# montekki/thaler-study

Hardware: AMD Instinct MI355X
Metric: field mul-adds/sec in sumcheck prover, n=28 vars (higher is better)
Workload: dtype u64

## Files before the change

thaler-study_amd/csrc/engine/abi_context.inc:

```


extern "C" int sc_field_from_modulus(uint64_t p, sc_field* out) {
  if (!out) return SC_ERR_ARG;
  sc::FieldParams fp;
  if (!sc::field_params_from_modulus(p, &fp)) return SC_ERR_ARG;
  out->p = fp.p;
  out->p_inv_neg = fp.p_inv_neg;
  out->r_mod_p = fp.r_mod_p;
  out->r2_mod_p = fp.r2_mod_p;
  return SC_OK;
}

static sc::FieldParams to_params(const sc_field* f) {
  sc::FieldParams fp;
  fp.p = f->p;
  fp.p_inv_neg = f->p_inv_neg;
  fp.r_mod_p = f->r_mod_p;
  fp.r2_mod_p = f->r2_mod_p;
  return fp;
}

extern "C" uint64_t sc_field_to_mont(const sc_field* f, uint64_t canonical) {
  HostField hf(to_params(f));
  return hf.mul(canonical % f->p, f->r2_mod_p);
// ... 73 lines not shown
  memset(ctx->h_tail, 0, kTailSlots * kTailSlotWords * sizeof(u64));
  SC_CREATE_HIP(hipHostGetDevicePointer((void**)&ctx->d_tail, ctx->h_tail, 0));
  for (int i = kTailSlots - 1; i >= 0; --i) ctx->tail_free.push_back(i);
  SC_CREATE_HIP(hipDeviceSynchronize());
  for (int i = 0; i < sc_ctx::kTimerRing; ++i) {
    SC_CREATE_HIP(hipEventCreate(&ctx->kt_ev[i][0]));
    SC_CREATE_HIP(hipEventCreate(&ctx->kt_ev[i][1]));
  }
#undef SC_CREATE_HIP
  *out = ctx;
  return SC_OK;
}

extern "C" int sc_ctx_destroy(sc_ctx* ctx) {
  if (!ctx) return SC_OK;
  if (is_multi(ctx)) return multi_destroy(ctx);
  (void)hipSetDevice(ctx->device);
  if (ctx->stream) (void)sync_stream(ctx);
  if (ctx->comm && g_rccl.CommDestroy) g_rccl.CommDestroy(ctx->comm);
  for (int q = 0; q < sc::kMaxPeers; ++q)
    if (ctx->peer_ipc_opened[q] && ctx->peer_base[q]) (void)hipIpcCloseMemHandle(ctx->peer_base[q]);
  if (ctx->peer_region) (void)hipFree(ctx->peer_region);
  for (auto& kv : ctx->pool_free) (void)hipFree(kv.second);
  for (auto& kv : ctx->pool_live) (void)hipFree(kv.first);
  if (ctx->d_partials) (void)hipFree(ctx->d_partials);
  if (ctx->d_wg_partials) (void)hipFree(ctx->d_wg_partials);
  if (ctx->d_wg_groups) (void)hipFree(ctx->d_wg_groups);
  if (ctx->d_wg_tickets) (void)hipFree(ctx->d_wg_tickets);
  if (ctx->d_gram_rows) (void)hipFree(ctx->d_gram_rows);
  if (ctx->d_sums) (void)hipFree(ctx->d_sums);
  if (ctx->h_sums) (void)hipHostFree(ctx->h_sums);
  if (ctx->h_mailbox) (void)hipHostFree(ctx->h_mailbox);
  if (ctx->h_tail) (void)hipHostFree(ctx->h_tail);
  if (ctx->h_points) (void)hipHostFree(ctx->h_points);
  if (ctx->d_points) (void)hipFree(ctx->d_points);
  for (u64* tw : ctx->d_rs_twiddles)
    if (tw) (void)hipFree(tw);
  for (u64* tw : ctx->d_rs_twist)
    if (tw) (void)hipFree(tw);
  if (ctx->d_xc_inv) (void)hipFree(ctx->d_xc_inv);
  if (ctx->h_batch_desc) (void)hipHostFree(ctx->h_batch_desc);
  if (ctx->h_batch) (void)hipHostFree(ctx->h_batch);
  if (ctx->d_ticket) (void)hipFree(ctx->d_ticket);
  for (int i = 0; i < sc_ctx::kTimerRing; ++i)
    for (int k = 0; k < 2; ++k)
      if (ctx->kt_ev[i][k]) (void)hipEventDestroy(ctx->kt_ev[i][k]);
  if (ctx->stream) (void)hipStreamDestroy(ctx->stream);
  delete ctx;
  return SC_OK;
}

extern "C" const char* sc_last_error(const sc_ctx* ctx) {
  return ctx ? ctx->err.c_str() : g_create_error.c_str();
}

static int prewarm(sc_ctx* ctx, size_t num_vars);

enum : unsigned { kOptBool = 1, kOptOff = 2, kOptPeer = 4 };
struct OptionSpec {
  const char* name;
  int sc_ctx::*member;
  int64_t lo, hi;
  unsigned flags;
};
const OptionSpec kOptions[] = {
    {"vars_per_pass", &sc_ctx::vars_per_pass, 1, 2, 0},
    {"first_pass_vars", &sc_ctx::first_pass_vars, 0, 4, 0},
    {"grid_pass", &sc_ctx::grid_pass, 0, 1, kOptBool},
    {"grid_log", &sc_ctx::grid_log, 0, 26, 0},
    {"grid_max_vars", &sc_ctx::grid_max_vars, 1, sc::kGridMaxVars, 0},
    {"grid_sharded", &sc_ctx::grid_sharded, 0, 1, kOptBool},
    {"grid_blocks", &sc_ctx::grid_blocks, 0, kWgMaxBlocks, 0},
    {"fold_dma", &sc_ctx::fold_dma, 0, 1, kOptBool},
    {"pipe32", &sc_ctx::pipe32, 0, 1, kOptBool},
    {"pipe32_log", &sc_ctx::pipe32_log, 11, 40, 0},
    {"gram_log", &sc_ctx::gram_log, 14, 40, kOptOff},
    {"wfold_log", &sc_ctx::wfold_log, 12, 40, kOptOff},
    {"wfold_min_log", &sc_ctx::wfold_min_log, 12, 40, 0},
    {"wfold5_min_log", &sc_ctx::wfold5_min_log, 12, 40, 0},
    {"wfold_always", &sc_ctx::wfold_always, 0, 1, kOptBool},
    {"wfold_slot_period", &sc_ctx::wfold_slot_period, -1, 1 << 24, 0},
    {"wfold_slot_width", &sc_ctx::wfold_slot_width, 0, 1 << 24, 0},
    {"wfold_slot_stagger", &sc_ctx::wfold_slot_stagger, 0, 1, kOptBool},
    {"matmul_path", &sc_ctx::matmul_path, 0, 2, 0},
    {"host_tail_log", &sc_ctx::host_tail_log, 0, kTailLogMax, 0},
    {"gp_host_log", &sc_ctx::gp_host_log, 0, sc::kGpHostLogMax, 0},
    {"gp_tree_lv", &sc_ctx::gp_tree_lv, 1, 3, 0},
    {"fr_host_log", &sc_ctx::fr_host_log, 0, sc::kFrHostLogMax, 0},
    {"fr_tree_lv", &sc_ctx::fr_tree_lv, 1, sc::kFrTreeLvMax, 0},
    {"tail_log", &sc_ctx::tail_log, 0, 40, 0},
    {"max_blocks", &sc_ctx::max_blocks, 1, INT64_MAX, 0},
    {"time_kernels", &sc_ctx::time_kernels, 0, 1, kOptBool},
    {"use_mailbox", &sc_ctx::use_mailbox, 0, 1, kOptBool},
    {"nt_load_log", &sc_ctx::nt_load_log, INT64_MIN, INT64_MAX, 0},
    {"nt_store_log", &sc_ctx::nt_store_log, INT64_MIN, INT64_MAX, 0},
    {"pool_contiguous", &sc_ctx::pool_contiguous, 0, 1, kOptBool},
    {"dbg_fold_grab", &sc_ctx::dbg_fold_grab, 0, 16, 0},
    {"rccl_timeout_ms", &sc_ctx::rccl_timeout_ms, 1, 3600000, 0},
    {"arena_log", &sc_ctx::arena_log, 4, 26, kOptPeer},
    {"peer_spin_ms", &sc_ctx::peer_spin_ms, 1, 600000, kOptPeer},
    {"peer_connect_ms", &sc_ctx::peer_connect_ms, 1, 3600000, kOptPeer},
    {"dbg_delay_ms", &sc_ctx::dbg_delay_ms, 0, 10000, kOptPeer},
    {"dbg_skip_tag", &sc_ctx::dbg_skip_tag, 0, 1, kOptBool | kOptPeer},
};
static const OptionSpec* find_option(const char* key) {
  for (const OptionSpec& o : kOptions)
    if (strcmp(o.name, key) == 0) return &o;
  return nullptr;
}

extern "C" int sc_ctx_set_option(sc_ctx* ctx, const char* key, int64_t value) {
  if (!ctx || !key) return SC_ERR_ARG;
  const std::string k(key);
  if (k == "prewarm") return value < 0 ? fail(ctx, SC_ERR_ARG, "prewarm: num_vars must be >= 0") : prewarm(ctx, (size_t)value);
  if (is_multi(ctx)) SC_TRY(multi_set_option(ctx, key, value));
  if (k == "stat_reset") {
    ctx->stat_wait_ns = ctx->stat_launch_ns = 0;
    ctx->pool_peak_words = ctx->pool_live_words;
    return SC_OK;
  }
  const OptionSpec* o = find_option(key);
  if (!o) return fail(ctx, SC_ERR_ARG, "unknown option '%s'", key);
  if (o->member == &sc_ctx::max_blocks && (value < 1 || value > (int64_t)ctx->partial_rows))
    return fail(ctx, SC_ERR_ARG, "max_blocks must be 1..%zu", ctx->partial_rows);
  if (!(o->flags & kOptBool) && (value < o->lo || value > o->hi) && !((o->flags & kOptOff) && value == 0))
    return fail(ctx, SC_ERR_ARG, "%s must be %s%lld..%lld", key, (o->flags & kOptOff) ? "0 (never) or " : "", (long long)o->lo, (long long)o->hi);
  if (o->member == &sc_ctx::arena_log && ctx->peer_region) return fail(ctx, SC_ERR_STATE, "arena_log must be set before sc_ctx_comm_peer_export");
  ctx->*o->member = (o->flags & kOptBool) ? (value ? 1 : 0) : (int)value;
  return SC_OK;
}

static int64_t pool_stat(const sc_ctx* ctx, size_t (*of)(const sc_ctx*)) {
  if (!is_multi(ctx)) return (int64_t)of(ctx);
  int64_t sum = 0;
  for (const sc_ctx* sub : ctx->subs) sum += (int64_t)of(sub);
  return sum;
}

extern "C" int sc_ctx_get_option(const sc_ctx* ctx, const char* key, int64_t* value) {
  if (!ctx || !key || !value) return SC_ERR_ARG;
  const std::string k(key);
  if (k == "stat_wait_ns") *value = (int64_t)(is_multi(ctx) ? ctx->subs[0]->stat_wait_ns : ctx->stat_wait_ns);
  else if (k == "stat_launch_ns") *value = (int64_t)(is_multi(ctx) ? ctx->subs[0]->stat_launch_ns : ctx->stat_launch_ns);
  else if (k == "stat_pool_live_blocks") *value = pool_stat(ctx, [](const sc_ctx* c) { return c->pool_live.size(); });
  else if (k == "stat_pool_live_words") *value = pool_stat(ctx, [](const sc_ctx* c) { return c->pool_live_words; });
  else if (k == "stat_pool_peak_words") *value = pool_stat(ctx, [](const sc_ctx* c) { return c->pool_peak_words; });
  else if (k == "transport") *value = (int64_t)ctx->transport;
  else if (k == "n_devices") *value = is_multi(ctx) ? (int64_t)ctx->subs.size() : 1;
  else if (k == "comm_nranks") {
    int n = ctx->world;
    if (ctx->transport == Transport::kRccl) {
      n = 0;
      if (!g_rccl.CommCount || !ctx->comm || g_rccl.CommCount(ctx->comm, &n) != ncclSuccess)
        return fail(ctx, SC_ERR_RCCL, "ncclCommCount failed");
    }
    *value = n;
  } else if (const OptionSpec* o = find_option(key)) {
    *value = ctx->*o->member;
  } else {
    return fail(ctx, SC_ERR_ARG, "unknown option '%s'", key);
  }
  return SC_OK;
}

extern "C" int sc_ctx_synchronize(sc_ctx* ctx) {
  if (!ctx) return SC_ERR_ARG;
  if (is_multi(ctx)) return multi_synchronize(ctx);
  SC_TRY(set_device(ctx));
  SC_HIP(ctx, sync_stream(ctx));
  return SC_OK;
}

extern "C" void* sc_ctx_stream(const sc_ctx* ctx) { return !ctx ? nullptr : (void*)(is_multi(ctx) ? ctx->subs[0]->stream : ctx->stream); }

extern "C" int sc_ctx_kernel_time(sc_ctx* ctx, double out[2], int reset) {
  if (!ctx || !out) return SC_ERR_ARG;
  if (is_multi(ctx)) {
    for (size_t d = 1; d < ctx->subs.size(); ++d) {
      double drop[2];
      (void)sc_ctx_kernel_time(ctx->subs[d], drop, reset);
    }
    return sc_ctx_kernel_time(ctx->subs[0], out, reset);
  }
  SC_TRY(set_device(ctx));
  drain_kernel_timers(ctx);
  out[0] = (double)ctx->kt_n;
  out[1] = ctx->kt_ms;
  if (reset) {
    ctx->kt_n = 0;
    ctx->kt_ms = 0.0;
  }
  return SC_OK;
}

extern "C" int sc_ctx_launch_log(sc_ctx* ctx, sc_launch_record* out, size_t cap, size_t* n_out, int reset) {
  if (!ctx || !n_out || (cap && !out)) return SC_ERR_ARG;
  if (is_multi(ctx)) {
    for (size_t d = 1; d < ctx->subs.size(); ++d) {
      size_t drop = 0;
      (void)sc_ctx_launch_log(ctx->subs[d], nullptr, 0, &drop, reset);
    }
    return sc_ctx_launch_log(ctx->subs[0], out, cap, n_out, reset);
  }
  SC_TRY(set_device(ctx));
  drain_kernel_timers(ctx);
  const size_t n = std::min(cap, ctx->launch_log.size());
  for (size_t i = 0; i < n; ++i) out[i] = ctx->launch_log[i];
  *n_out = ctx->launch_log.size();
  if (reset) ctx->launch_log.clear();
// ... 3 lines not shown
```

thaler-study_amd/csrc/engine/launch.inc:

```

namespace {


#define SC_DISPATCH_FIELD(ctx, F, f, ...)      \
  do {                                         \
    if ((ctx)->gold) {                         \
      typedef sc::GoldilocksMont F;            \
      F f((ctx)->fp);                          \
      __VA_ARGS__;                             \
    } else {                                   \
      typedef sc::MontGeneric F;               \
      F f((ctx)->fp);                          \
      __VA_ARGS__;                             \
    }                                          \
  } while (0)

template <int V>
using IntC = std::integral_constant<int, V>;
template <int... Vs, class Fn>
void with_const(int v, Fn&& fn) {
  (void)((v == Vs && (fn(IntC<Vs>{}), true)) || ...);
}
template <class Fn>
void with_bool(bool b, Fn&& fn) {
// ... 205 lines not shown
    SC_HIP(ctx, hipGetLastError());
  }
  ctx->mailbox_seq += 1;
  return SC_OK;
}

bool in_tail(const sc_ctx* ctx, const u64* p) { return p && ctx->d_tail && p >= ctx->d_tail && p < ctx->d_tail + kTailSlots * kTailSlotWords; }

int launch_pass(sc_ctx* ctx, int kf, int ks, const u64* A, const u64* B, u64* A2, u64* B2, const u64* r,
                int log_in, bool across_ranks, bool* from_mailbox) {
  if (kf < 0 || kf > 4 || ks < 1 || ks > 3 || (ks == 3 && kf != 0) || (kf == 4 && (ks != 2 || log_in < 12)) || log_in < kf + ks)
    return fail(ctx, SC_ERR_ARG, "launch_pass: kf=%d ks=%d log_in=%d", kf, ks, log_in);
  const sc::FoldW fw = make_weights<sc::FoldW>(ctx, r, kf);
  size_t n_units = (size_t)1 << (log_in - kf - ks);
  const bool pipe32 = kf == 3 && ks == 2 && ctx->pipe32 && n_units % sc::kWave == 0 && log_in >= ctx->pipe32_log;
  const size_t bs = (size_t)sc::pass_block_threads(kf, ks, pipe32 ? 4 : 0);
  int grid = (int)std::min<size_t>(std::max<size_t>((n_units + bs - 1) / bs, 1), (size_t)ctx->max_blocks);
  grid = std::min(grid, pipe32 ? pipe32_resident_blocks(ctx) : pass_resident_blocks(ctx, kf, ks));
  if (kf > 0 && in_tail(ctx, A2) && (grid != 1 || ((size_t)1 << (log_in - kf)) > (size_t)sc::kWave))
    return fail(ctx, SC_ERR_STATE, "launch_pass: a pass_kernel launch of %d blocks would hand 2^%d-entry tables to the host with plain stores", grid,
                log_in - kf);
  const sc::PassOut out = next_pass_out(ctx, across_ranks, challenge_digest(r, kf, ks, log_in), from_mailbox);
  SC_TRY(timer_begin(ctx, SC_KIND_PASS, kf, ks, log_in, (u64)16 << log_in, kf > 0 ? (u64)16 << (log_in - kf) : 0));
  SC_DISPATCH_FIELD(ctx, F, f, launch_pass_t<F>(ctx, f, kf, ks, A, B, A2, B2, fw, n_units, grid, log_in, out, pipe32));
  SC_TRY(commit_pass_out(ctx, out, grid));
  SC_TRY(timer_end(ctx));
  return SC_OK;
}

int wait_mailbox(sc_ctx* ctx, u64 seq);

int check_exchange(sc_ctx* ctx, const char* what) {
  const u64 err = __atomic_load_n(ctx->h_mailbox + sc::kMailboxErr, __ATOMIC_ACQUIRE);
  if (err == 0) return SC_OK;
  if (err & (u64)sc::kXchgTimeout) {
    poison(ctx);
    return fail(ctx, SC_ERR_RCCL, "peer exchange: a rank's %s did not arrive within %d ms (rank %d waited for rank %d at tag %u; that rank's "
                "slot held tag ..%04x)", what, ctx->peer_spin_ms, ctx->rank, (int)((err >> 8) & 0xFF), ctx->xchg_tag, (unsigned)((err >> 16) & 0x3FFF));
  }
  return fail(ctx, SC_ERR_STATE, "the ranks of this sharded prover were given different challenges");
}

int launch_grid_pass(sc_ctx* ctx, int kf, int ks, const u64* A, const u64* B, u64* A2, u64* B2, const u64* r, int log_in, bool across_ranks) {
  if (kf < 0 || kf > sc::kGridMaxVars || ks < 1 || ks > sc::kGridMaxVars || log_in < kf + ks)
    return fail(ctx, SC_ERR_ARG, "launch_grid_pass: kf=%d ks=%d log_in=%d", kf, ks, log_in);
  if (!ctx->use_mailbox) return fail(ctx, SC_ERR_STATE, "launch_grid_pass needs the host mailbox");
  const sc::GridW gw = make_weights<sc::GridW>(ctx, r, kf);
  const size_t n_out = (size_t)1 << (log_in - kf);
  const int resident = std::min(resident_grid(ctx, ctx->gold ? kernel_ptr(&sc::wgrid_pass_kernel<sc::GoldilocksMont, 5, false>)
                                                             : kernel_ptr(&sc::wgrid_pass_kernel<sc::MontGeneric, 5, false>),
                                              sc::kBlock, 2 * ctx->num_cus),
                                kWgMaxBlocks);
  constexpr size_t kWaves = sc::kBlock / sc::kWave;
  const size_t n_iter = (n_out + sc::kWgEntries - 1) / sc::kWgEntries;
  const size_t cap = ctx->grid_blocks > 0 ? (size_t)std::min(ctx->grid_blocks, resident) : (size_t)resident;
  const int grid = (int)std::max<size_t>(1, std::min<size_t>((n_iter + kWaves - 1) / kWaves, cap));
  const sc::WgOut wo = next_wide_out(ctx, across_ranks, challenge_digest(r, kf, ks, log_in), true, in_tail(ctx, A2));
  SC_TRY(timer_begin(ctx, SC_KIND_GRID_PASS, kf, ks, log_in, (u64)16 << log_in, kf > 0 ? (u64)16 << (log_in - kf) : 0));
  const bool pf = (kf == 0 || kf == 2) && n_iter > (size_t)grid * kWaves;
  SC_DISPATCH_FIELD(ctx, F, f, with_bool(pf, [&](auto PF) {
    with_const<1, 2, 3, 4, 5>(ks, [&](auto KS) {
      hipLaunchKernelGGL((sc::wgrid_pass_kernel<F, KS, PF>), dim3(grid), dim3(sc::kBlock), 0, ctx->stream, f, A, B, A2, B2, gw, kf, n_out, wo);
    });
  }));
  return commit_wide_out(ctx, wo, pow3(ks));
}
bool wfold_has(int kf, int ks) { return (kf == 4 && ks == 5) || (kf == 5 && ks >= 3 && ks <= 5); }
int wfold_resident_blocks(sc_ctx* ctx) {
  const void* fn = ctx->gold ? kernel_ptr(&sc::wfold_pass_kernel<sc::GoldilocksMont, 4, 5, true>)
                             : kernel_ptr(&sc::wfold_pass_kernel<sc::MontGeneric, 4, 5, true>);
  return std::min(resident_grid(ctx, fn, sc::kWfThreads, ctx->num_cus), kWgMaxBlocks);
}
int launch_wfold_pass(sc_ctx* ctx, int kf, int ks, const u64* A, const u64* B, u64* A2, u64* B2, const u64* r, int log_in, bool across_ranks) {
  if (log_in < 12 || !A2 || !B2 || !wfold_has(kf, ks)) return fail(ctx, SC_ERR_ARG, "launch_wfold_pass: kf=%d ks=%d log_in=%d", kf, ks, log_in);
  if (!ctx->use_mailbox) return fail(ctx, SC_ERR_STATE, "launch_wfold_pass needs the host mailbox");
  const sc::FoldW fw = make_weights<sc::FoldW>(ctx, r, 4);
  const u64 r_top = kf == 5 ? r[4] : 0;
  const size_t n_tiles = (size_t)1 << (log_in - 12);
  const int grid = (int)std::max<size_t>(1, std::min<size_t>(std::min<size_t>(n_tiles, (size_t)wfold_resident_blocks(ctx)), (size_t)ctx->max_blocks));
  const sc::WgOut wo = next_wide_out(ctx, across_ranks, challenge_digest(r, kf, ks, log_in) ^ 0x77666f6cu, true, false);
  SC_TRY(timer_begin(ctx, SC_KIND_WFOLD_PASS, kf, ks, log_in, (u64)16 << log_in, (u64)16 << (log_in - kf)));
  sc::WfSlots sl;
  if (ctx->wfold_slot_period < 0) {
    sl.period = (kf == 4 && log_in >= 25) ? 2400u : 0u;
    sl.width = 600u;
  } else {
    sl.period = (unsigned)ctx->wfold_slot_period;
    sl.width = (unsigned)ctx->wfold_slot_width;
    sl.stagger = (unsigned)ctx->wfold_slot_stagger;
  }
  SC_DISPATCH_FIELD(ctx, F, f, with_bool(log_in >= ctx->nt_load_log, [&](auto NT) {
    with_bool(sl.period != 0, [&](auto SLOTS) {
      auto go = [&](auto KF, auto KS) {
        hipLaunchKernelGGL((sc::wfold_pass_kernel<F, KF, KS, NT, SLOTS>), dim3(grid), dim3(sc::kWfThreads), 0, ctx->stream, f, A, B, A2, B2, fw, r_top,
                           n_tiles, wo, sl);
      };
      if (kf == 4) go(IntC<4>{}, IntC<5>{});
      else with_const<3, 4, 5>(ks, [&](auto KS) { go(IntC<5>{}, KS); });
    });
  }));
  return commit_wide_out(ctx, wo, pow3(ks));
}

constexpr int kGramK = 4;
constexpr int kGramMaxBlocks = 1024;
int gram_workspace(sc_ctx* ctx) {
  if (ctx->d_gram_rows) return SC_OK;
  const size_t bytes = (size_t)kGramMaxBlocks * sc::kGramRowWords * sizeof(u64) + 64;
  u64* p = nullptr;
  SC_HIP(ctx, hipMalloc(&p, bytes));
  hipError_t e = hipMemsetAsync(p, 0, bytes, ctx->stream);
  const int lds = sc::kGramStages * sc::kGramStageBytes;
  const void* fns[4] = {reinterpret_cast<const void*>(&sc::gram_pass_kernel<sc::GoldilocksMont, kGramK, true>),
                        reinterpret_cast<const void*>(&sc::gram_pass_kernel<sc::GoldilocksMont, kGramK, false>),
                        reinterpret_cast<const void*>(&sc::gram_pass_kernel<sc::MontGeneric, kGramK, true>),
                        reinterpret_cast<const void*>(&sc::gram_pass_kernel<sc::MontGeneric, kGramK, false>)};
  for (int i = 0; i < 4 && e == hipSuccess; ++i) e = hipFuncSetAttribute(fns[i], hipFuncAttributeMaxDynamicSharedMemorySize, lds);
  if (e != hipSuccess) {
    (void)hipFree(p);
    SC_HIP(ctx, e);
  }
  ctx->d_gram_rows = p;
  return SC_OK;
}
int launch_gram_pass(sc_ctx* ctx, const u64* A, const u64* B, int log_in, bool across_ranks) {
  typedef sc::GramGeo<kGramK> G;
  if (!ctx->use_mailbox) return fail(ctx, SC_ERR_STATE, "launch_gram_pass needs the host mailbox");
  const size_t len = (size_t)1 << log_in;
  if (len < (size_t)G::kEntriesPerStep * sc::kGramStages) return fail(ctx, SC_ERR_ARG, "launch_gram_pass: 2^%d entries are too few", log_in);
  const size_t n_steps = len / G::kEntriesPerStep;
  size_t blocks = 1;
  while (blocks * 2 <= (size_t)std::min(std::min(ctx->num_cus, ctx->max_blocks), kGramMaxBlocks)) blocks *= 2;
  size_t n_partials = std::min(blocks, n_steps / sc::kGramStages);
  while (n_steps / n_partials > (size_t)G::kMaxSteps) n_partials *= 2;
  const size_t spp = n_steps / n_partials;
  const int grid = (int)std::min(blocks, n_partials);
  SC_TRY(gram_workspace(ctx));
  const sc::WgOut wo = next_wide_out(ctx, across_ranks, challenge_digest(nullptr, 0, kGramK, log_in) ^ 0x6772616du, false, false);
  unsigned* ticket = reinterpret_cast<unsigned*>(ctx->d_gram_rows + (size_t)kGramMaxBlocks * sc::kGramRowWords);
  SC_TRY(timer_begin(ctx, SC_KIND_GRAM_PASS, 0, kGramK, log_in, (u64)16 << log_in, (u64)grid * sc::kGramRowWords * sizeof(u64)));
  const unsigned char* a8 = reinterpret_cast<const unsigned char*>(A);
  const unsigned char* b8 = reinterpret_cast<const unsigned char*>(B);
  const int lds = sc::kGramStages * sc::kGramStageBytes;
  SC_DISPATCH_FIELD(ctx, F, f, with_bool(log_in >= ctx->nt_load_log, [&](auto NT) {
    hipLaunchKernelGGL((sc::gram_pass_kernel<F, kGramK, NT>), dim3(grid), dim3(sc::kGramThreads), lds, ctx->stream, f, a8, b8,
                       (unsigned)n_partials, (unsigned)spp, ctx->d_gram_rows, ticket, wo);
  }));
  return commit_wide_out(ctx, wo, pow3(kGramK));
}

int collect_grid(sc_ctx* ctx, int ks, bool across_ranks, u64* out) {
  SC_TRY(wait_mailbox(ctx, ctx->mailbox_seq));
  const int cells = pow3(ks);
  const u64* wide = ctx->h_mailbox + sc::kMailboxWide;
  if (!across_ranks) {
    for (int c = 0; c < cells; ++c) out[c] = wide[c];
    return SC_OK;
  }
  HostField hf(ctx->fp);
  if (ctx->transport == Transport::kHost) {
    std::vector<u64> limbs(2 * (size_t)cells);
    for (int c = 0; c < cells; ++c) {
      limbs[2 * c] = wide[c] & 0xFFFFFFFFull;
      limbs[2 * c + 1] = wide[c] >> 32;
    }
    if (ctx->host_allreduce(ctx->host_user, limbs.data(), limbs.size()) != 0)
      return fail(ctx, SC_ERR_RCCL, "host all-reduce callback failed");
    for (int c = 0; c < cells; ++c) out[c] = hf.recombine(limbs[2 * c], limbs[2 * c + 1]);
    return SC_OK;
  }
  if (ctx->transport == Transport::kPeer) SC_TRY(check_exchange(ctx, "sums"));
  for (int c = 0; c < cells; ++c) out[c] = hf.recombine(wide[2 * c], wide[2 * c + 1]);
// ... 20 lines not shown
```

thaler-study_amd/csrc/kernels/grid_pass.hpp:

```cpp
#pragma once

namespace sc {

constexpr int kGridChunk = 256;
constexpr int kGridMaxVars = 5;
constexpr int kGridMaxCells = 243;
constexpr int kMailboxWide = 64;
constexpr int kMailboxWords = kMailboxWide + 512;
constexpr int kWgEntries = 32;
constexpr int kWgGroupBlocks = 32;
struct GridW {
  u64 w[1 << kGridMaxVars];
};
struct WgOut {
  u64* partials;
  u64* group_rows;
  unsigned* tickets;
  u64* mailbox;
  u64 seq;
  u64* limbs_dev;
  PeerX px;
  int host_out = 0;
};
template <class F, int KF>
// ... 279 lines not shown
    return;
  }
  if (tid < CELLS) __hip_atomic_store(out.mailbox + kMailboxWide + tid, total, __ATOMIC_RELAXED, __HIP_MEMORY_SCOPE_SYSTEM);
  asm volatile("s_waitcnt vmcnt(0)" ::: "memory");
  __syncthreads();
  if (tid == 0) __hip_atomic_store(out.mailbox + kMailboxSeq, out.seq, __ATOMIC_RELEASE, __HIP_MEMORY_SCOPE_SYSTEM);
}

template <class F, int KS>
__device__ __forceinline__ void wgrid_finish(const F& f, u64 total, const WgOut& out) {
  constexpr int kPow3[6] = {1, 3, 9, 27, 81, 243};
  constexpr int cells = kPow3[KS];
  __shared__ int lds_flag;
  const int tid = threadIdx.x;
  if (gridDim.x > 1) {
    const int n_blocks = gridDim.x, group = blockIdx.x / kWgGroupBlocks, n_groups = (n_blocks + kWgGroupBlocks - 1) / kWgGroupBlocks;
    const int group_size = min(kWgGroupBlocks, n_blocks - group * kWgGroupBlocks);
    if (tid < cells)
      __hip_atomic_store(out.partials + (size_t)blockIdx.x * kGridChunk + tid, total, __ATOMIC_RELAXED, __HIP_MEMORY_SCOPE_AGENT);
    asm volatile("s_waitcnt vmcnt(0)" ::: "memory");
    __syncthreads();
    if (tid == 0) {
      const unsigned t = __hip_atomic_fetch_add(out.tickets + 1 + group, 1u, __ATOMIC_RELAXED, __HIP_MEMORY_SCOPE_AGENT);
      const int last = (t == (unsigned)group_size - 1) ? 1 : 0;
      if (last) {
        __builtin_amdgcn_fence(__ATOMIC_ACQUIRE, "agent");
        asm volatile("s_waitcnt vmcnt(0)" ::: "memory");
      }
      lds_flag = last;
    }
    __syncthreads();
    if (!lds_flag) return;
    total = 0;
    if (tid < cells) {
      u64 x[kWgGroupBlocks];
#pragma unroll
      for (int q = 0; q < kWgGroupBlocks; ++q)
        x[q] = (q < group_size) ? __hip_atomic_load(out.partials + (size_t)(group * kWgGroupBlocks + q) * kGridChunk + tid, __ATOMIC_RELAXED,
                                                    __HIP_MEMORY_SCOPE_AGENT)
                                : 0;
#pragma unroll
      for (int q = 0; q < kWgGroupBlocks; ++q) total = f.add(total, x[q]);
    }
    if (n_groups > 1) {
      __syncthreads();
      if (tid < cells)
        __hip_atomic_store(out.group_rows + (size_t)group * kGridChunk + tid, total, __ATOMIC_RELAXED, __HIP_MEMORY_SCOPE_AGENT);
      asm volatile("s_waitcnt vmcnt(0)" ::: "memory");
      __syncthreads();
      if (tid == 0) {
        const unsigned t = __hip_atomic_fetch_add(out.tickets, 1u, __ATOMIC_RELAXED, __HIP_MEMORY_SCOPE_AGENT);
        const int last = (t == (unsigned)n_groups - 1) ? 1 : 0;
        if (last) {
          __builtin_amdgcn_fence(__ATOMIC_ACQUIRE, "agent");
          asm volatile("s_waitcnt vmcnt(0)" ::: "memory");
        }
        lds_flag = last;
      }
      __syncthreads();
      if (!lds_flag) return;
      total = 0;
      if (tid < cells) {
        u64 x[kWgGroupBlocks];
#pragma unroll
        for (int q = 0; q < kWgGroupBlocks; ++q)
          x[q] = (q < n_groups) ? __hip_atomic_load(out.group_rows + (size_t)q * kGridChunk + tid, __ATOMIC_RELAXED, __HIP_MEMORY_SCOPE_AGENT) : 0;
#pragma unroll
        for (int q = 0; q < kWgGroupBlocks; ++q) total = f.add(total, x[q]);
      }
    }
    if (tid <= n_groups) __hip_atomic_store(out.tickets + tid, 0u, __ATOMIC_RELAXED, __HIP_MEMORY_SCOPE_AGENT);
  }
  publish_cells<cells>(out, total);
}

template <class F, int KS, bool PF>
__global__ void __launch_bounds__(kBlock)
wgrid_pass_kernel(F f, const u64* __restrict__ A, const u64* __restrict__ B, u64* __restrict__ A2, u64* __restrict__ B2,
                  GridW gw, int kf, size_t n_out, WgOut out) {
  const u64 total = wgrid_body<F, KS, PF>(f, A, B, A2, B2, gw, kf, n_out, out.host_out != 0);
  wgrid_finish<F, KS>(f, total, out);
}

#define SC_WFOLD_SLOTS 1
struct WfSlots {
  unsigned period = 0;
  unsigned width = 0;
  unsigned stagger = 0;
};
constexpr int kWfThreads = 512;
template <class F, int KF, int KS, bool NT, bool SLOTS = false>
__global__ void __launch_bounds__(kWfThreads)
wfold_pass_kernel(F f, const u64* __restrict__ A, const u64* __restrict__ B, u64* __restrict__ A2, u64* __restrict__ B2, FoldW fw,
                  u64 r_top, size_t n_tiles, WgOut out, WfSlots sl) {
  static_assert(KF == 4 || KF == 5, "four or five pending challenges");
  static_assert(KS >= 1 && KS <= 5, "one to five rounds");
  constexpr int OUT = 4, NPS = 8, NP = 32;
  constexpr int OUTS = kWave >> (KF - 4);
  constexpr int TILE_OUT = OUT * OUTS;
  constexpr int NPO = TILE_OUT / (2 * kWave);
  constexpr int kWaves = kWfThreads / kWave;
  constexpr int kPow3[6] = {1, 3, 9, 27, 81, 243};
  constexpr int cells = kPow3[KS], G = 1 << KS, gpi = kWgEntries >> KS, pairs = gpi * cells;
  constexpr int kRegionWords = 1024 + 512 + 512;
  __shared__ u64 lds_all[kWaves * kRegionWords];
  __shared__ int cell_of[kWgEntries], suffix_of[kWgEntries];
  __shared__ unsigned lds_next;
  constexpr unsigned kNoTile = ~0u;
  __shared__ unsigned lds_slots[4];
  __shared__ unsigned lds_wave[kWaves][2];
  typedef __attribute__((address_space(3))) u64 lds_u64;
  const int tid = threadIdx.x, lane = tid & (kWave - 1), wave = tid / kWave;
  auto lds_word = [](const unsigned* p) -> unsigned {
    return (unsigned)__builtin_amdgcn_readfirstlane((int)*(const volatile unsigned*)p);
  };
  if constexpr (SLOTS) {
    if (tid == 0) {
      lds_slots[0] = sl.period;
      lds_slots[1] = sl.width;
      lds_slots[2] = sl.stagger ? (blockIdx.x & 7u) * (sl.period >> 3) : 0u;
    }
    if (lane == 0) {
      lds_wave[wave][0] = kNoTile;
      lds_wave[wave][1] = ((unsigned)wall_clock64() + (sl.stagger ? (blockIdx.x & 7u) * (sl.period >> 3) : 0u) - sl.width) / sl.period;
    }
  }
  if (tid < kWgEntries) {
    int c = 0, u = 0, p3 = 1;
    for (int m = 0; m < KS; ++m) {
      c += ((tid >> (KS - 1 - m)) & 1) * p3;
      u += ((tid >> m) & 1) * p3;
      p3 *= 3;
    }
    cell_of[tid] = c;
    suffix_of[tid] = u;
  }
  if (tid == 0) lds_next = 0;
  __syncthreads();
  ull2* const reg = reinterpret_cast<ull2*>(lds_all + (size_t)wave * kRegionWords);
  u64* const xchg = lds_all + (size_t)wave * kRegionWords + 1024;
  u64* const ef = xchg + 512;
  const int tbl = lane >> 5, ent = lane & (kWgEntries - 1);
  const int slot = tbl * kGridChunk + (ent >> KS) * cells + cell_of[ent & (G - 1)];
  unsigned step[KS][3];
#pragma clang loop unroll(full)
  for (int j = 0; j < KS; ++j) {
    const int low = KS - 1 - j, pj = kPow3[j], stride = kPow3[low], items = (gpi * pj) << low;
    const unsigned inv = (1u << 20) / (unsigned)pj + 1u;
#pragma clang loop unroll(full)
    for (int q = 0; q < 3; ++q) {
      const int idx = lane + kWave * q;
      unsigned d = 0;
      if (idx < 2 * items) {
        const int tb = idx >= items ? 1 : 0, id = idx - tb * items;
        const int sfx = id & ((1 << low) - 1), t = id >> low;
        const int g = (int)(((unsigned)t * inv) >> 20), pp = t - g * pj;
        d = 0x80000000u | (unsigned)(size_t)(lds_u64*)(ef + tb * kGridChunk + g * cells + pp * 3 * stride + suffix_of[sfx]);
      }
      step[j][q] = d;
    }
  }
  typename F::Acc acc[4];
#pragma unroll
  for (int k = 0; k < 4; ++k) f.acc_zero(acc[k]);

  const ull2* __restrict__ Ap = reinterpret_cast<const ull2*>(A);
  const ull2* __restrict__ Bp = reinterpret_cast<const ull2*>(B);
  ull2* __restrict__ A2p = reinterpret_cast<ull2*>(A2);
  ull2* __restrict__ B2p = reinterpret_cast<ull2*>(B2);
  const int rot = wave & 3;
  auto next_tile = [&]() -> size_t {
    unsigned c = 0;
    if (lane == 0) c = __hip_atomic_fetch_add(&lds_next, 1u, __ATOMIC_RELAXED, __HIP_MEMORY_SCOPE_WORKGROUP);
    return (size_t)__builtin_amdgcn_readfirstlane(c) * gridDim.x + blockIdx.x;
  };
  auto load_sub = [&](const ull2* __restrict__ T, size_t tile, int o, ull2 (&p)[NPS]) {
    const ull2* src = T + tile * kWave * NP + (size_t)o * NPS * kWave + lane;
#pragma unroll
    for (int k = 0; k < NPS; ++k) p[k] = ld16<NT>(src + k * kWave);
  };
  auto stash = [&](const ull2 (&p)[NPS]) {
#pragma unroll
    for (int k = 0; k < NPS; ++k) reg[swz_slot<NPS>(64 * k + lane)] = p[k];
  };
  auto fold16 = [&]() -> u64 {
    typename F::Acc3 sacc;
    f.acc3_zero(sacc);
#pragma unroll
    for (int m = 0; m < NPS; ++m) {
      const ull2 x = reg[swz_slot<NPS>(NPS * lane + m)];
      f.acc3_mac(sacc, x.x, fw.w[2 * m]);
      f.acc3_mac(sacc, x.y, fw.w[2 * m + 1]);
    }
    const u64 h = f.acc3_get(sacc);
    if constexpr (KF == 5) {
      const u64 hn = __shfl_xor(h, 1);
      return f.add(h, f.mul(r_top, f.sub(hn, h)));
    } else {
      return h;
    }
  };
  auto put = [&](u64* dst, int o, u64 x) {
    if constexpr (KF == 5) {
      if ((lane & 1) == 0) dst[OUTS * o + (lane >> 1)] = x;
    } else {
      dst[OUTS * o + lane] = x;
    }
  };
  auto grid_group = [&](int grp) {
    ef[slot] = xchg[kWave * OUT * tbl + kWgEntries * grp + ent];
    wave_lds_sync();
#pragma clang loop unroll(full)
    for (int j = 0; j < KS; ++j) {
      const int st = kPow3[KS - 1 - j];
#pragma clang loop unroll(full)
      for (int q = 0; q < 3; ++q) {
        if (2 * ((gpi * kPow3[j]) << (KS - 1 - j)) > kWave * q) {
          const unsigned d = step[j][q];
          if (d != 0) {
            lds_u64* const x = (lds_u64*)(size_t)(d & 0x7FFFFFFFu);
            x[2 * st] = f.sub(x[st], x[0]);
          }
        }
      }
      wave_lds_sync();
    }
#pragma unroll
    for (int k = 0; k < 4; ++k) {
      const int p = lane + kWave * k;
      if (p < pairs) f.acc_mac(acc[k], ef[p], ef[kGridChunk + p]);
    }
    wave_lds_sync();
  };
  ull2 held[2 * NPO];
  auto store_held = [&](unsigned t) {
#pragma unroll
    for (int k = 0; k < NPO; ++k) {
      const size_t q = (size_t)t * kWave * NPO + (size_t)k * kWave + lane;
      st16<false>(A2p + q, held[2 * k]);
      st16<false>(B2p + q, held[2 * k + 1]);
    }
    lds_wave[wave][0] = kNoTile;
  };
  ull2 pa[NPS], pb[NPS];
  size_t tile = next_tile();
  if (tile < n_tiles) {
    load_sub(Ap, tile, rot, pa);
    load_sub(Bp, tile, rot, pb);
  }
  while (tile < n_tiles) {
    const size_t next = next_tile();
#pragma unroll
    for (int i = 0; i < OUT; ++i) {
      const int o = (i + rot) & 3, no = (i + 1 + rot) & 3;
      if constexpr (SLOTS) {
        const unsigned period = lds_word(&lds_slots[0]), width = lds_word(&lds_slots[1]);
        const unsigned t = (unsigned)wall_clock64() + lds_word(&lds_slots[2]);
        const unsigned ht = lds_word(&lds_wave[wave][0]);
        if (ht != kNoTile && t % period < width) store_held(ht);
        if (wave == 0 && blockIdx.x < 8) {
          const unsigned k = (t - width) / period;
          if (k != lds_word(&lds_wave[0][1])) asm volatile("buffer_wbl2 sc1" ::: "memory");
          lds_wave[0][1] = k;
        }
      }
      stash(pa);
      wave_lds_sync();
      if (i + 1 < OUT) load_sub(Ap, tile, no, pa);
      else if (next < n_tiles) load_sub(Ap, next, no, pa);
      const u64 xa = fold16();
      wave_lds_sync();
      stash(pb);
      wave_lds_sync();
      if (i + 1 < OUT) load_sub(Bp, tile, no, pb);
      else if (next < n_tiles) load_sub(Bp, next, no, pb);
      const u64 xb = fold16();
      put(xchg, o, xa);
      put(xchg + kWave * OUT, o, xb);
      wave_lds_sync();
#pragma unroll 1
      for (int g = 0; g < OUTS / kWgEntries; ++g) grid_group(o * (OUTS / kWgEntries) + g);
    }
    {
      const ull2* xo = reinterpret_cast<const ull2*>(xchg);
      const size_t o0 = tile * kWave * NPO;
      if (SLOTS && lds_word(&lds_slots[1]) != 0) {
        const unsigned ht = lds_word(&lds_wave[wave][0]);
        if (ht != kNoTile) store_held(ht);
#pragma unroll
        for (int k = 0; k < NPO; ++k) {
          held[2 * k] = xo[kWave * k + lane];
          held[2 * k + 1] = xo[kWave * OUT / 2 + kWave * k + lane];
        }
        lds_wave[wave][0] = (unsigned)tile;
      } else {
#pragma unroll
        for (int k = 0; k < NPO; ++k) {
          const size_t q = o0 + (size_t)k * kWave + lane;
          st16<false>(A2p + q, xo[kWave * k + lane]);
          st16<false>(B2p + q, xo[kWave * OUT / 2 + kWave * k + lane]);
        }
      }
    }
    wave_lds_sync();
    if constexpr (!SLOTS) {
      if (wave == 0 && blockIdx.x < 8) asm volatile("buffer_wbl2 sc1" ::: "memory");
    }
    tile = next;
  }
  if constexpr (SLOTS) {
    const unsigned ht = lds_word(&lds_wave[wave][0]);
    if (ht != kNoTile) store_held(ht);
  }
  __syncthreads();
  u64* const red = lds_all;
#pragma unroll
  for (int k = 0; k < 4; ++k) {
    const int p = lane + kWave * k;
    red[wave * kGridChunk + p] = (p < pairs) ? f.acc_get(acc[k]) : 0;
  }
  __syncthreads();
  u64 total = 0;
  if (tid < cells) {
    for (int w = 0; w < kWaves; ++w)
      for (int g = 0; g < gpi; ++g) total = f.add(total, red[w * kGridChunk + g * cells + tid]);
  }
  wgrid_finish<F, KS>(f, total, out);
}

template <class F>
__global__ void __launch_bounds__(kBlock)
rank_pass_kernel(F f, const u64* __restrict__ A, const u64* __restrict__ B, u64* __restrict__ A2, u64* __restrict__ B2, GridW gw, int kf,
                 WgOut out) {
  const PeerX& px = out.px;
  __shared__ u64 ta[kMaxPeers], tb[kMaxPeers];
  __shared__ int worst;
  const int tid = threadIdx.x;
  const size_t par = (size_t)(px.tag & 1u) * kMaxPeers * kInboxWords;
  int err = 0;
  if (tid == 0) worst = 0;
  if (tid < 2) {
    const u64* __restrict__ src = tid ? B : A;
    const int fan = 1 << kf;
    u64 v = 0;
    for (int c = 0; c < fan; ++c) v = f.add(v, f.mul(src[c], gw.w[c]));
    const ull2 pair = {((u64)px.tag << 32) | (v & 0xFFFFFFFFull), ((u64)px.tag << 32) | (v >> 32)};
    const size_t mine = par + (size_t)px.rank * kInboxWords + kInboxWide + 2 * (size_t)tid;
    for (int q = 0; q < px.world; ++q) st16_system(px.inbox[q] + mine, pair);
  }
  if (tid == 2) {
    const u64 g = ((u64)px.tag << 32) | (u64)px.digest;
    for (int q = 0; q < px.world; ++q)
      __hip_atomic_store(px.inbox[q] + par + (size_t)px.rank * kInboxWords + kInboxDigest, g, __ATOMIC_RELAXED, __HIP_MEMORY_SCOPE_SYSTEM);
  }
  const unsigned long long t0 = wall_clock64();
  if (tid < 3 * px.world) {
    const int r = tid / 3, what = tid % 3;
    const u64* base = px.inbox[px.rank] + par + (size_t)r * kInboxWords;
    unsigned spins = 0;
    while (true) {
      if (what < 2) {
        const ull2 g = ld16_system(base + kInboxWide + 2 * what);
        if ((unsigned)(g.x >> 32) == px.tag && (unsigned)(g.y >> 32) == px.tag) {
          const u64 v = (g.x & 0xFFFFFFFFull) | (g.y << 32);
          (what ? tb : ta)[r] = v;
          break;
        }
      } else {
        const u64 g = __hip_atomic_load(base + kInboxDigest, __ATOMIC_RELAXED, __HIP_MEMORY_SCOPE_SYSTEM);
        if ((unsigned)(g >> 32) == px.tag) {
          err = ((unsigned)g != px.digest) ? kXchgDigest : 0;
          break;
        }
      }
      if ((++spins & 31) == 0 && wall_clock64() - t0 > px.spin_ticks) {
        err = kXchgTimeout | (r << 8);
        break;
      }
      __builtin_amdgcn_s_sleep(1);
    }
  }
  __syncthreads();
  if (err) atomicMax(&worst, err);
  __syncthreads();
  if (worst == 0) {
    if (tid < px.world) {
      A2[tid] = ta[tid];
      B2[tid] = tb[tid];
    }
    int g = 0;
    while ((1 << g) < px.world) ++g;
    int cells = 1;
    for (int j = 0; j < g; ++j) cells *= 3;
    if (tid < cells) {
      int d[3] = {0, 0, 0};
      int c = tid;
// ... 33 lines not shown
```

thaler-study_amd/csrc/sumcheck_hip.hip:

```cpp
#include <dlfcn.h>
#include <hip/hip_runtime.h>
#include <rccl/rccl.h>

#include <algorithm>
#include <chrono>
#include <cstdarg>
#include <cstdio>
#include <cstring>
#include <atomic>
#include <condition_variable>
#include <functional>
#include <map>
#include <memory>
#include <mutex>
#include <new>
#include <set>
#include <string>
#include <thread>
#include <type_traits>
#include <vector>

#include "../../include/sumcheck_hip.h"
#include "kernels.hpp"

// ... 19 lines not shown

RcclApi g_rccl;
std::string g_create_error;

bool load_rccl(std::string* why) {
  if (g_rccl.handle) return true;
  const char* chosen = getenv("SC_RCCL_LIBRARY");
  const char* names[] = {"librccl.so.1", "librccl.so", "/opt/rocm/lib/librccl.so.1"};
  void* h = nullptr;
  if (chosen && *chosen) {
    h = dlopen(chosen, RTLD_NOW | RTLD_LOCAL);
    if (!h) {
      *why = std::string("dlopen(SC_RCCL_LIBRARY=") + chosen + ") failed: " + dlerror();
      return false;
    }
  } else {
    for (const char* n : names) {
      h = dlopen(n, RTLD_NOW | RTLD_LOCAL);
      if (h) break;
    }
  }
  if (!h) {
    *why = std::string("dlopen(librccl) failed: ") + dlerror();
    return false;
  }
  RcclApi a;
  a.handle = h;
  a.GetUniqueId = (decltype(a.GetUniqueId))dlsym(h, "ncclGetUniqueId");
  a.CommInitRank = (decltype(a.CommInitRank))dlsym(h, "ncclCommInitRank");
  a.CommDestroy = (decltype(a.CommDestroy))dlsym(h, "ncclCommDestroy");
  a.CommCount = (decltype(a.CommCount))dlsym(h, "ncclCommCount");
  a.AllReduce = (decltype(a.AllReduce))dlsym(h, "ncclAllReduce");
  a.AllGather = (decltype(a.AllGather))dlsym(h, "ncclAllGather");
  a.GetErrorString = (decltype(a.GetErrorString))dlsym(h, "ncclGetErrorString");
  a.CommAbort = (decltype(a.CommAbort))dlsym(h, "ncclCommAbort");
  a.CommGetAsyncError = (decltype(a.CommGetAsyncError))dlsym(h, "ncclCommGetAsyncError");
  if (!a.GetUniqueId || !a.CommInitRank || !a.CommDestroy || !a.AllReduce || !a.AllGather) {
    *why = "librccl is missing a required symbol";
    return false;
  }
  g_rccl = a;
  return true;
}

enum class Transport { kNone, kRccl, kHost, kPeer, kLocal };
constexpr int kMaxSubs = 8;
constexpr int kTailLogMax = 12;
constexpr int kTailSoftLog = 11;
constexpr int kTailEntries = 1 << kTailLogMax;
constexpr int kTailSmallLog = 5;
constexpr int kTailSlots = 32;
constexpr size_t kTailSlotWords = 2 * (size_t)kTailEntries;
constexpr int kWgMaxBlocks = 1024;

}

struct sc_ctx {
  sc::FieldParams fp;
  bool gold = false;
  int device = 0;
  hipStream_t stream = nullptr;
  mutable std::string err;
  mutable bool poisoned = false;

  int vars_per_pass = 2;
  int first_pass_vars = 0;
  int grid_pass = 1;
  int grid_log = 20;
  int grid_max_vars = 5;
  int grid_sharded = 1;
  int grid_blocks = 0;
  u64* d_wg_partials = nullptr;
  u64* d_wg_groups = nullptr;
  unsigned* d_wg_tickets = nullptr;
  u64* d_gram_rows = nullptr;
  int fold_dma = 1;
  int pipe32 = 1, pipe32_log = 20;
  int gram_log = 21;
  int host_tail_log = kTailLogMax;
  int wfold_log = 40;
  int wfold_min_log = 21;
  int wfold5_min_log = 24;
  int wfold_always = 0;
  int wfold_slot_period = -1, wfold_slot_width = 0, wfold_slot_stagger = 0;
  int matmul_path = 0;
  int gp_host_log = 10;
  int gp_tree_lv = sc::kGpTreeLv;
  int fr_host_log = 9;
  int fr_tree_lv = sc::kFrTreeLv;
  int tail_log = 16;
  int max_blocks = 768;
  int num_cus = 256;
  std::map<const void*, int> resident_grid;
  int time_kernels = 0;
  uint64_t stat_wait_ns = 0, stat_launch_ns = 0;
  int nt_load_log = 22;
  int nt_store_log = 25;

  u64* d_partials = nullptr;
  u64* d_sums = nullptr;
  u64* h_sums = nullptr;
  size_t partial_rows = 0;
  unsigned* d_ticket = nullptr;
  bool fold_lds_allowed[4][2] = {};
  unsigned ticket_base = 0;
  u64* h_mailbox = nullptr;
  u64* d_mailbox = nullptr;
  u64 mailbox_seq = 0;
  int use_mailbox = 1;

  std::multimap<size_t, u64*> pool_free;
  std::map<u64*, size_t> pool_live;
  size_t pool_live_words = 0, pool_peak_words = 0;

  Transport transport = Transport::kNone;
  int rank = 0, world = 1, log_world = 0;
  ncclComm_t comm = nullptr;
  sc_allreduce_fn host_allreduce = nullptr;
  sc_allgather_fn host_allgather = nullptr;
  void* host_user = nullptr;
  u64* peer_region = nullptr;
  size_t peer_region_words = 0;
  bool peer_exported = false;
  u64* peer_base[sc::kMaxPeers] = {};
  bool peer_ipc_opened[sc::kMaxPeers] = {};
  int arena_log = 17;
  unsigned xchg_tag = 0;
  unsigned xchg_next = 0;
  unsigned gather_count = 0;
  int peer_spin_ms = 2000;
  int rccl_timeout_ms = 30000;
  mutable bool comm_failed = false;
  int peer_connect_ms = 120000;
  int dbg_delay_ms = 0;
  int dbg_skip_tag = 0;
  int dbg_fold_grab = 0;
  int pool_contiguous = 0;

  std::vector<sc_ctx*> subs;
  sc_ctx* parent = nullptr;
  struct MultiRuntime* mrt = nullptr;
  u64* h_tail = nullptr;
  u64* d_tail = nullptr;
  std::vector<int> tail_free;
  u64* h_points = nullptr;
  u64* d_points = nullptr;
  void* h_batch_desc = nullptr;
  size_t batch_desc_bytes = 0;
  u64* h_batch = nullptr;
  u64* d_batch = nullptr;
  size_t batch_words = 0;
  bool rs_root_known = false;
  int rs_two_adicity = 0;
  u64 rs_w_max = 0;
  u64* d_rs_twiddles[15] = {};
  u64* d_rs_twist[25] = {};
  std::set<const void*> lds_allowed;
  u64* d_xc_inv = nullptr;

  static constexpr int kTimerRing = 64;
  static constexpr size_t kLaunchLogCap = 1 << 16;
  hipEvent_t kt_ev[kTimerRing][2] = {};
  sc_launch_record kt_meta[kTimerRing] = {};
  int kt_used = 0;
  double kt_ms = 0.0;
  long kt_n = 0;
  std::vector<sc_launch_record> launch_log;
// ... 304 lines not shown
```

Before: 902.2 billion.

## Double-buffer held fold tiles and widen wall-clock store slots in wfold pass

The slotted wfold kernel now holds up to two finished output tiles per wave in registers instead of one. It flushes them to global memory only inside wall-clock time windows, and the default slot period doubles so write bursts land less often. Optional extra slot checks within each output iteration are added behind a 'looks' option, and the default path keeps one check per iteration. The aim is to group output stores into synchronized bursts so they interfere less with streaming loads. The cost is more registers per thread, which may lower occupancy, plus extra LDS bookkeeping.

```diff
diff --git a/thaler-study_amd/csrc/engine/abi_context.inc b/thaler-study_amd/csrc/engine/abi_context.inc
--- a/thaler-study_amd/csrc/engine/abi_context.inc
+++ b/thaler-study_amd/csrc/engine/abi_context.inc
@@ -179,6 +179,8 @@
     {"wfold_slot_period", &sc_ctx::wfold_slot_period, -1, 1 << 24, 0},
     {"wfold_slot_width", &sc_ctx::wfold_slot_width, 0, 1 << 24, 0},
     {"wfold_slot_stagger", &sc_ctx::wfold_slot_stagger, 0, 1, kOptBool},
+    {"wfold_slot_hold", &sc_ctx::wfold_slot_hold, 1, 2, 0},
+    {"wfold_slot_looks", &sc_ctx::wfold_slot_looks, 4, 16, 0},
     {"matmul_path", &sc_ctx::matmul_path, 0, 2, 0},
     {"host_tail_log", &sc_ctx::host_tail_log, 0, kTailLogMax, 0},
     {"gp_host_log", &sc_ctx::gp_host_log, 0, sc::kGpHostLogMax, 0},
@@ -222,6 +224,7 @@
     return fail(ctx, SC_ERR_ARG, "max_blocks must be 1..%zu", ctx->partial_rows);
   if (!(o->flags & kOptBool) && (value < o->lo || value > o->hi) && !((o->flags & kOptOff) && value == 0))
     return fail(ctx, SC_ERR_ARG, "%s must be %s%lld..%lld", key, (o->flags & kOptOff) ? "0 (never) or " : "", (long long)o->lo, (long long)o->hi);
+  if (o->member == &sc_ctx::wfold_slot_looks && value != 4 && value != 8 && value != 16) return fail(ctx, SC_ERR_ARG, "wfold_slot_looks must be 4, 8 or 16");
   if (o->member == &sc_ctx::arena_log && ctx->peer_region) return fail(ctx, SC_ERR_STATE, "arena_log must be set before sc_ctx_comm_peer_export");
   ctx->*o->member = (o->flags & kOptBool) ? (value ? 1 : 0) : (int)value;
   return SC_OK;
diff --git a/thaler-study_amd/csrc/engine/launch.inc b/thaler-study_amd/csrc/engine/launch.inc
--- a/thaler-study_amd/csrc/engine/launch.inc
+++ b/thaler-study_amd/csrc/engine/launch.inc
@@ -311,12 +311,15 @@
   SC_TRY(timer_begin(ctx, SC_KIND_WFOLD_PASS, kf, ks, log_in, (u64)16 << log_in, (u64)16 << (log_in - kf)));
   sc::WfSlots sl;
   if (ctx->wfold_slot_period < 0) {
-    sl.period = (kf == 4 && log_in >= 25) ? 2400u : 0u;
+    sl.period = (kf == 4 && log_in >= 25) ? 4800u : 0u;
     sl.width = 600u;
+    sl.hold = 2u;
   } else {
     sl.period = (unsigned)ctx->wfold_slot_period;
     sl.width = (unsigned)ctx->wfold_slot_width;
     sl.stagger = (unsigned)ctx->wfold_slot_stagger;
+    sl.hold = (unsigned)ctx->wfold_slot_hold;
+    sl.looks = (unsigned)ctx->wfold_slot_looks;
   }
   SC_DISPATCH_FIELD(ctx, F, f, with_bool(log_in >= ctx->nt_load_log, [&](auto NT) {
     with_bool(sl.period != 0, [&](auto SLOTS) {
diff --git a/thaler-study_amd/csrc/kernels/grid_pass.hpp b/thaler-study_amd/csrc/kernels/grid_pass.hpp
--- a/thaler-study_amd/csrc/kernels/grid_pass.hpp
+++ b/thaler-study_amd/csrc/kernels/grid_pass.hpp
@@ -385,11 +385,13 @@
   wgrid_finish<F, KS>(f, total, out);
 }
 
-#define SC_WFOLD_SLOTS 1
+#define SC_WFOLD_SLOTS 2
 struct WfSlots {
   unsigned period = 0;
   unsigned width = 0;
   unsigned stagger = 0;
+  unsigned hold = 1;
+  unsigned looks = 4;
 };
 constexpr int kWfThreads = 512;
 template <class F, int KF, int KS, bool NT, bool SLOTS = false>
@@ -410,8 +412,8 @@
   __shared__ int cell_of[kWgEntries], suffix_of[kWgEntries];
   __shared__ unsigned lds_next;
   constexpr unsigned kNoTile = ~0u;
-  __shared__ unsigned lds_slots[4];
-  __shared__ unsigned lds_wave[kWaves][2];
+  __shared__ unsigned lds_slots[6];
+  __shared__ unsigned lds_wave[kWaves][4];
   typedef __attribute__((address_space(3))) u64 lds_u64;
   const int tid = threadIdx.x, lane = tid & (kWave - 1), wave = tid / kWave;
   auto lds_word = [](const unsigned* p) -> unsigned {
@@ -422,9 +424,11 @@
       lds_slots[0] = sl.period;
       lds_slots[1] = sl.width;
       lds_slots[2] = sl.stagger ? (blockIdx.x & 7u) * (sl.period >> 3) : 0u;
+      lds_slots[3] = sl.looks;
+      lds_slots[4] = sl.hold;
     }
     if (lane == 0) {
-      lds_wave[wave][0] = kNoTile;
+      lds_wave[wave][0] = lds_wave[wave][2] = kNoTile;
       lds_wave[wave][1] = ((unsigned)wall_clock64() + (sl.stagger ? (blockIdx.x & 7u) * (sl.period >> 3) : 0u) - sl.width) / sl.period;
     }
   }
@@ -535,15 +539,35 @@
     }
     wave_lds_sync();
   };
-  ull2 held[2 * NPO];
-  auto store_held = [&](unsigned t) {
+  ull2 held[2][2 * NPO];
+  auto store_held = [&](const ull2 (&h)[2 * NPO], int set, unsigned t) {
 #pragma unroll
     for (int k = 0; k < NPO; ++k) {
       const size_t q = (size_t)t * kWave * NPO + (size_t)k * kWave + lane;
-      st16<false>(A2p + q, held[2 * k]);
-      st16<false>(B2p + q, held[2 * k + 1]);
-    }
-    lds_wave[wave][0] = kNoTile;
+      st16<false>(A2p + q, h[2 * k]);
+      st16<false>(B2p + q, h[2 * k + 1]);
+    }
+    lds_wave[wave][2 * set] = kNoTile;
+  };
+  auto store_all = [&]() {
+    const unsigned h0 = lds_word(&lds_wave[wave][0]), h1 = lds_word(&lds_wave[wave][2]);
+    if (h1 < h0) {
+      store_held(held[1], 1, h1);
+      if (h0 != kNoTile) store_held(held[0], 0, h0);
+    } else {
+      if (h0 != kNoTile) store_held(held[0], 0, h0);
+      if (h1 != kNoTile) store_held(held[1], 1, h1);
+    }
+  };
+  auto look = [&]() {
+    const unsigned period = lds_word(&lds_slots[0]), width = lds_word(&lds_slots[1]);
+    const unsigned t = (unsigned)wall_clock64() + lds_word(&lds_slots[2]);
+    if (t % period < width) store_all();
+    if (wave == 0 && blockIdx.x < 8) {
+      const unsigned k = (t - width) / period;
+      if (k != lds_word(&lds_wave[0][1])) asm volatile("buffer_wbl2 sc1" ::: "memory");
+      lds_wave[0][1] = k;
+    }
   };
   ull2 pa[NPS], pb[NPS];
   size_t tile = next_tile();
@@ -556,16 +580,10 @@
 #pragma unroll
     for (int i = 0; i < OUT; ++i) {
       const int o = (i + rot) & 3, no = (i + 1 + rot) & 3;
+      unsigned looks = 4;
       if constexpr (SLOTS) {
-        const unsigned period = lds_word(&lds_slots[0]), width = lds_word(&lds_slots[1]);
-        const unsigned t = (unsigned)wall_clock64() + lds_word(&lds_slots[2]);
-        const unsigned ht = lds_word(&lds_wave[wave][0]);
-        if (ht != kNoTile && t % period < width) store_held(ht);
-        if (wave == 0 && blockIdx.x < 8) {
-          const unsigned k = (t - width) / period;
-          if (k != lds_word(&lds_wave[0][1])) asm volatile("buffer_wbl2 sc1" ::: "memory");
-          lds_wave[0][1] = k;
-        }
+        look();
+        looks = lds_word(&lds_slots[3]);
       }
       stash(pa);
       wave_lds_sync();
@@ -573,6 +591,9 @@
       else if (next < n_tiles) load_sub(Ap, next, no, pa);
       const u64 xa = fold16();
       wave_lds_sync();
+      if constexpr (SLOTS) {
+        if (__builtin_expect(looks >= 8, 0)) look();
+      }
       stash(pb);
       wave_lds_sync();
       if (i + 1 < OUT) load_sub(Bp, tile, no, pb);
@@ -581,21 +602,40 @@
       put(xchg, o, xa);
       put(xchg + kWave * OUT, o, xb);
       wave_lds_sync();
+      if constexpr (SLOTS) {
+        if (__builtin_expect(looks >= 16, 0)) look();
+      }
 #pragma unroll 1
-      for (int g = 0; g < OUTS / kWgEntries; ++g) grid_group(o * (OUTS / kWgEntries) + g);
+      for (int g = 0; g < OUTS / kWgEntries; ++g) {
+        if constexpr (SLOTS) {
+          if (__builtin_expect(g > 0 && looks >= 16, 0)) look();
+        }
+        grid_group(o * (OUTS / kWgEntries) + g);
+      }
     }
     {
       const ull2* xo = reinterpret_cast<const ull2*>(xchg);
       const size_t o0 = tile * kWave * NPO;
       if (SLOTS && lds_word(&lds_slots[1]) != 0) {
-        const unsigned ht = lds_word(&lds_wave[wave][0]);
-        if (ht != kNoTile) store_held(ht);
-#pragma unroll
-        for (int k = 0; k < NPO; ++k) {
-          held[2 * k] = xo[kWave * k + lane];
-          held[2 * k + 1] = xo[kWave * OUT / 2 + kWave * k + lane];
-        }
-        lds_wave[wave][0] = (unsigned)tile;
+        const unsigned h0 = lds_word(&lds_wave[wave][0]), h1 = lds_word(&lds_wave[wave][2]);
+        const bool first = lds_word(&lds_slots[4]) < 2 || h0 == kNoTile || (h1 != kNoTile && h0 < h1);
+        if (first) {
+          if (h0 != kNoTile) store_held(held[0], 0, h0);
+#pragma unroll
+          for (int k = 0; k < NPO; ++k) {
+            held[0][2 * k] = xo[kWave * k + lane];
+            held[0][2 * k + 1] = xo[kWave * OUT / 2 + kWave * k + lane];
+          }
+          lds_wave[wave][0] = (unsigned)tile;
+        } else {
+          if (h1 != kNoTile) store_held(held[1], 1, h1);
+#pragma unroll
+          for (int k = 0; k < NPO; ++k) {
+            held[1][2 * k] = xo[kWave * k + lane];
+            held[1][2 * k + 1] = xo[kWave * OUT / 2 + kWave * k + lane];
+          }
+          lds_wave[wave][2] = (unsigned)tile;
+        }
       } else {
 #pragma unroll
         for (int k = 0; k < NPO; ++k) {
@@ -611,10 +651,7 @@
     }
     tile = next;
   }
-  if constexpr (SLOTS) {
-    const unsigned ht = lds_word(&lds_wave[wave][0]);
-    if (ht != kNoTile) store_held(ht);
-  }
+  if constexpr (SLOTS) store_all();
   __syncthreads();
   u64* const red = lds_all;
 #pragma unroll
diff --git a/thaler-study_amd/csrc/sumcheck_hip.hip b/thaler-study_amd/csrc/sumcheck_hip.hip
--- a/thaler-study_amd/csrc/sumcheck_hip.hip
+++ b/thaler-study_amd/csrc/sumcheck_hip.hip
@@ -125,7 +125,7 @@
   int wfold_min_log = 21;
   int wfold5_min_log = 24;
   int wfold_always = 0;
-  int wfold_slot_period = -1, wfold_slot_width = 0, wfold_slot_stagger = 0;
+  int wfold_slot_period = -1, wfold_slot_width = 0, wfold_slot_stagger = 0, wfold_slot_hold = 1, wfold_slot_looks = 4;
   int matmul_path = 0;
   int gp_host_log = 10;
   int gp_tree_lv = sc::kGpTreeLv;
```

Result: no change. 902.4 billion, median of 4 (+0.0%).
